# hydradarpa/kalman-hydra

Measured on AMD Instinct MI355X. Metric: frames/sec (Brox flow + EKF update) at 1024^2, higher is better.
Workload: dtype f32 (flow, renders) / f64 (EKF sums and state)

## Files before the change

### kalman-hydra_amd/csrc/chol_flow_kernels.h

```cpp
#pragma once
#include <hip/hip_runtime.h>
#include "dense_kernels.h"

#define FLOW_NT 256
#ifdef HM_STAMP
#define HM_CHAIN_STAMP(c, k) do { if (g_stamp && (threadIdx.x & 63) == 0) g_stamp[(size_t)(4096 + (c)) * 8 + (k)] = clock64(); } while (0)
#else
#define HM_CHAIN_STAMP(c, k) do { } while (0)
#endif
#define FLOW_SENTINEL 0x7FF8DEADBEEF0001ull
#define FLOW_POLL_LIMIT 4000000


__device__ __forceinline__ unsigned long long flow_ld_bits(const double *p)
{
    return __hip_atomic_load((const unsigned long long *)p, __ATOMIC_RELAXED, __HIP_MEMORY_SCOPE_AGENT);
}
__device__ __forceinline__ void flow_st(double *p, double v)
{
    __hip_atomic_store((unsigned long long *)p, (unsigned long long)__double_as_longlong(v), __ATOMIC_RELAXED,
                       __HIP_MEMORY_SCOPE_AGENT);
}

__device__ __forceinline__ void flow_fill_row(const FlowArgs &a, int row, int t, int nt)
{
    const double s = __longlong_as_double((long long)FLOW_SENTINEL);
    if (row < a.nrows) {
        const int upto = row < a.nb * DNB ? (row / DNB) * DNB : a.n;
        for (int j = t; j < upto; j += nt) a.L[(size_t)row * a.n + j] = s;
    }
    if (row < a.n) {
        const int upto = min(a.n, (row / DNB + 1) * DNB);
        for (int j = t; j < upto; j += nt) a.Tinv[(size_t)row * a.n + j] = s;
    }
}
#define FLOW_FILL_WGS 32
__device__ __forceinline__ void flow_fill_blocks(const FlowArgs &a, int t, int nt)
{
    const double s = __longlong_as_double((long long)FLOW_SENTINEL);
    for (int i = t; i < a.nb * DNB * DNB; i += nt) a.Lt[i] = s;
    for (int i = t; i < 3 * a.nb * DNB * DNB; i += nt) a.P[i] = s;
    if (t == 0) a.ctl[0] = 0;
}
__global__ __launch_bounds__(256) void k_flow_fill(FlowArgs a)
{
    if ((int)blockIdx.x >= a.nrows) flow_fill_blocks(a, ((int)blockIdx.x - a.nrows) * 256 + threadIdx.x, 256 * FLOW_FILL_WGS);
    else flow_fill_row(a, blockIdx.x, threadIdx.x, 256);
}

struct FlowBlock {
    const double *src;
    int ld, nr, nc;
    double (*dst)[DNB + 1];
};

__device__ __forceinline__ bool flow_fetch2(const FlowBlock &b0, const FlowBlock &b1, bool two, unsigned *ctl, bool hot = false)
{
    const int t = threadIdx.x;
    __shared__ int s_ok;
    double v0[4], v1[4];
    int patient = 0;
    for (int tries = 0;; tries++) {
        int ok0 = 1, ok1 = 1;
#pragma unroll
        for (int q = 0; q < 4; q++) {
            const int e = t + FLOW_NT * q, i = e / DNB, j = e % DNB;
            unsigned long long x0 = 0, x1 = 0;
            if (i < b0.nr && j < b0.nc) x0 = flow_ld_bits(b0.src + (size_t)i * b0.ld + j);
            if (two && i < b1.nr && j < b1.nc) x1 = flow_ld_bits(b1.src + (size_t)i * b1.ld + j);
            ok0 &= x0 != FLOW_SENTINEL;
// ... 404 lines not shown
```

### kalman-hydra_amd/csrc/ctx.h

```cpp
#pragma once
#include "hm_common.h"
#include "hm_types.h"
#include <chrono>
#include <cmath>
#include <condition_variable>
#include <functional>
#include <mutex>
#include <thread>
#include <vector>

struct Helper {
    std::thread th;
    std::mutex m;
    std::condition_variable cv;
    std::function<int()> job;
    bool posted = false, busy = false, quit = false;
    int rc = HM_OK;
    char err[512] = "";
    void run()
    {
        std::unique_lock<std::mutex> lk(m);
        for (;;) {
            cv.wait(lk, [&] { return quit || posted; });
            if (quit) return;
// ... 209 lines not shown
    long long n4_ticket = 0;
    bool n4_pending = false;
    int newton_fail = 0;
    hipEvent_t ev_n4 = nullptr, ev_pm = nullptr;
    bool n4_ready = false;
    bool chain_pending = false;
    std::vector<double> chain_pred, chain_proj;
    int chain_its = 0, chain_moved = 0;
    double *pin_blk = nullptr;
    std::thread worker;
    bool worker_active;
    int worker_rc;
    char worker_err[512];
    int chol_flow = 1, flow_wgs = 192;
    int flow_stall = 0;
    int speculate = 1;
    double *d_flowP;
    unsigned *d_flowctl;
    hipStream_t stream2;
    hipStream_t stream4 = nullptr;
    hipEvent_t ev_tail = nullptr;
    bool tail_on_stream4 = false;
    int tail_split = 1;
    int *d_nbars, *d_nvoff, *d_nvbar, *d_ninfo;
    double *d_nl0, *d_nX;
    bool newton_ready = false;
    int *d_ids[3];
    int *d_labels;
    int4 *d_lbox;
    double *d_lout;
    std::vector<double> h_lout;
    int2 *d_outline;
    int *d_outline_cnt;
    uint8_t *d_pm_mask;
    uint8_t *d_pm_flag = nullptr;
    uint8_t *d_pm_pruned = nullptr;
    Ccl ccl = {nullptr, nullptr, nullptr, nullptr, nullptr, 0, 0};
    double *d_pm_X = nullptr;
    double *pin_pm = nullptr;
    std::vector<double> pmv;
    int *d_pm_done = nullptr;
    long long pm_ticket = 0;
    bool pm_ready = false;
    bool outline_ready = false;
    const uint8_t *prepared_mask = nullptr;
    hipEvent_t ev_outline = nullptr;
    hipEvent_t ev_m0 = nullptr;
    ViewState view;
    BodyState body;
    StrainState strain;
    RecState rec;
};

static inline hipError_t alloc_targets(HmOwner &own, Targets &t, size_t n)
{
    hipError_t e = own.alloc(&t.acc, n * sizeof(int));
    if (e == hipSuccess) e = own.alloc(&t.fx, n * sizeof(float));
    if (e == hipSuccess) e = own.alloc(&t.fy, n * sizeof(float));
    if (e == hipSuccess) e = own.alloc(&t.cnt, n * sizeof(int));
    return e;
}

static int helper_join(hm_ctx *h)
{
    if (h->helper_used) {
        const int rc = h->helper.wait();
        if (rc != HM_OK) { hm_set_error("%s", h->helper.err); return rc; }
    }
    return HM_OK;
}
// ... 76 lines not shown
    for (int i = 0; i < n_bars; i++) {
        const int p = bars[2 * i], q = bars[2 * i + 1];
        bar[fill[p]] = i; other[fill[p]++] = q;
        bar[fill[q]] = i; other[fill[q]++] = p;
    }
}

static inline void spring_blocks(int n_bars, const int32_t *bars, const double *l0, double kappa, const double *X, double *blk)
{
    for (int i = 0; i < n_bars; i++) {
        const int a = bars[2 * i], b = bars[2 * i + 1];
        const double dx = X[2 * a] - X[2 * b], dy = X[2 * a + 1] - X[2 * b + 1];
        const double l = std::sqrt(dx * dx + dy * dy);
        const double k = kappa * (1.0 - l0[i] / l), c = kappa * l0[i] / (l * l * l);
        blk[3 * i] = k + c * dx * dx; blk[3 * i + 1] = c * dx * dy; blk[3 * i + 2] = k + c * dy * dy;
    }
}

__attribute__((visibility("hidden"))) void ekf_queue_setup_all(hipStream_t st, const Mesh &m, const double *d_X, TriSetup *d_setup);
__attribute__((visibility("hidden"))) void ekf_queue_render(hipStream_t st, const Mesh &m, const double *d_X, const TriSetup *d_setup,
                                                            const Targets &out, const int *d_labels, int *d_ids);
__attribute__((visibility("hidden"))) void ekf_queue_fpft(hipStream_t st, const double *src, double *FP, double *dst, int N,
                                                          const SpringTopo &tp, double a, double s, double eps_F);
__attribute__((visibility("hidden"))) void ekf_queue_chol_flow(hipStream_t st, const FlowArgs &a, int wgs, bool fill);

__attribute__((visibility("hidden"))) int body_map_build(hm_ctx *h);
__attribute__((visibility("hidden"))) int body_stats_queue_add(hm_ctx *h, const uint8_t *d_reg);
__attribute__((visibility("hidden"))) int body_rec_slot(hm_ctx *h, const char *who, uint8_t **dst);
__attribute__((visibility("hidden"))) int body_rec_queue_copy(hm_ctx *h, uint8_t *dst);
```

### kalman-hydra_amd/csrc/ekf.hip

```cpp
#include "ctx.h"
#include "ekf_kernels.h"
#include "dense_kernels.h"
#include "chol_flow_kernels.h"
#include "project_kernels.h"
#include "predict_kernels.h"
#include <algorithm>
#include <atomic>
#include <chrono>
#include <cmath>
#include <cstring>
#include <set>
#include <thread>
#include <utility>
#include <vector>


static int hb_wait(hipStream_t st, const double *blk, size_t first, size_t n, unsigned long long stamp, double *out, const char *who)
{
    const volatile unsigned long long *canary = (const volatile unsigned long long *)blk + 2 * (first + n - 1);
    const auto t_start = std::chrono::steady_clock::now();
    const auto t_yield = t_start + std::chrono::microseconds(700), t_give_up = t_start + std::chrono::milliseconds(20);
    bool polite = false;
    for (int spin = 0;; spin++) {
        if ((canary[0] ^ canary[1]) == stamp && hb_take(blk, first, n, stamp, out)) return HM_OK;
// ... 226 lines not shown
    return HM_OK;
}
#endif

#define TUNE_SET(field) [](hm_ctx *h, long long v) { h->field = (decltype(h->field))v; }
static const struct TuneKey {
    const char *key;
    long long lo, hi;
    int step;
    void (*set)(hm_ctx *, long long);
    const char *must;
} tune_keys[] = {
    {"measure_split", 1, MEAS_VSPLIT_MAX, 1, TUNE_SET(vsplit), nullptr},
    {"edge_split", 1, MEAS_VSPLIT_MAX, 1, TUNE_SET(esplit), nullptr},
    {"chol_flow", 0, 1, 1, TUNE_SET(chol_flow), "must be 0 (one launch per block step) or 1 (one persistent launch)"},
    {"chol_flow_wgs", 2, 2048, 1, TUNE_SET(flow_wgs), "must be in 2..2048 (the chain workgroup and at least one task workgroup)"},
    {"render_rows", 8, 16, 8, TUNE_SET(render_rows), "must be 8 or 16"},
    {"chol_flow_stall", 0, 100000, 1, TUNE_SET(flow_stall), nullptr},
    {"result_delay", 0, 5000, 1, TUNE_SET(result_delay), "must be in 0..5000 (microseconds)"},
    {"tail_async", 0, 1, 1, TUNE_SET(tail_async), "must be 0 or 1"},
    {"tail_split", 0, 1, 1, TUNE_SET(tail_split), "must be 0 or 1"},
    {"newton_fail", 0, 1, 1, TUNE_SET(newton_fail), "must be 0 or 1"},
    {"speculate", 0, 1, 1, TUNE_SET(speculate), "must be 0 or 1"},
    {"body_stats_cap", 1, BODY_STATS_CAP, 1, TUNE_SET(body.stats_cap), nullptr},
    {"body_rec_chunk", 0, INT32_MAX, 1, TUNE_SET(rec.chunk), "must be >= 0 (0: the default size)"},
    {"rec_tp_frames", 1, REC_TP_MAX, 1, TUNE_SET(rec.tp_frames), nullptr},
    {"rec_bl_frames", 1, REC_BL_MAX, 1, TUNE_SET(rec.bl_frames), nullptr},
    {"rec_res_frames", 1, REC_RES_MAX, 1, TUNE_SET(rec.res_frames), nullptr},
    {"rec_map_frames", 1, REC_MAP_MAX, 1, TUNE_SET(rec.map_frames), nullptr},
    {"rec_null_frames", 1, REC_NULL_MAX, 1, TUNE_SET(rec.null_frames), nullptr},
    {"rec_tm_frames", 1, REC_TM_MAX, 1, TUNE_SET(rec.tm_frames), nullptr},
    {"rec_gram_bytes", 64, REC_GRAM_BYTES_MAX, 64, TUNE_SET(rec.gram_bytes), "must be a multiple of 64 in 64..131008"},
    {"rec_scratch_bytes", 1, 1 << 30, 1, TUNE_SET(rec.scr_bytes), nullptr},
    {"rec_ev_bytes", 1, 1ll << 34, 1, TUNE_SET(rec.ev_bytes), nullptr},
};
#undef TUNE_SET
static const TuneKey *tune_find(const char *key)
{
    for (const TuneKey &k : tune_keys)
        if (!strcmp(key, k.key)) return &k;
    return nullptr;
}
static int tune_set(hm_ctx *h, const char *key, long long value)
{
    const TuneKey *k = tune_find(key);
    HM_ARG(k != nullptr, "hm_ctx_tune: unknown key '%s'", key);
// ... 149 lines not shown
    h->prepared_mask = nullptr;
    return HM_OK;
}

static int render_dev(hm_ctx *h, const double *dX, Targets t)
{
    Mesh m = {h->W, h->H, h->N, h->T, h->d_tri, h->d_uv, h->d_tex};
    hipLaunchKernelGGL(k_setup_all, dim3(hm_cdiv(h->T, 64)), dim3(64), 0, h->stream, m, dX, h->d_setup);
    hipLaunchKernelGGL((k_render<0>), dim3(hm_cdiv(h->W, EKF_TILE), hm_cdiv(h->H, EKF_TILE)), dim3(EKF_TILE, EKF_TILE), 0,
                       h->stream, m, dX, h->d_setup, t, (const int *)nullptr, (int *)nullptr);
    HM_HIP(hipGetLastError());
    return HM_OK;
}

static int render_into(hm_ctx *h, const double *X, Targets t)
{
    HM_HIP(hipMemcpyAsync(h->d_X, X, (size_t)4 * h->N * sizeof(double), hipMemcpyHostToDevice, h->stream));
    return render_dev(h, h->d_X, t);
}

static void measure_args(hm_ctx *h, const double *dX, double deltaX, int masked, MeasureArgs &a);
static int render_strips(const hm_ctx *h) { return hm_cdiv(h->W, RI_W) * hm_cdiv(h->H, h->render_rows); }

static int render_iter(hm_ctx *h, const double *dX, Targets t, bool with_err, int masked, bool regions, double deltaX)
{
    IterRenderArgs r;
    r.m = Mesh{h->W, h->H, h->N, h->T, h->d_tri, h->d_uv, h->d_tex};
    r.X = dX;
    r.out = t;
    r.o = Obs{h->o_yim, masked ? h->d_yfxm : h->o_yfx, masked ? h->d_yfym : h->o_yfy, h->o_ym};
    r.raw_fx = h->o_yfx; r.raw_fy = h->o_yfy;
    r.partial = h->d_tpart;
    r.tiles_x = hm_cdiv(h->W, RI_W); r.tiles_y = hm_cdiv(h->H, h->render_rows);
    const int nstrips = r.tiles_x * r.tiles_y;
    r.with_err = with_err ? 1 : 0;
    r.n_regions = regions ? h->N : 0;
    MeasureArgs a;
    measure_args(h, dX, deltaX, masked, a);
    if (h->render_rows == 8) hipLaunchKernelGGL((k_render_iter<8>), dim3(r.n_regions + nstrips), dim3(256), 0, h->stream, r, a, h->d_area);
    else hipLaunchKernelGGL((k_render_iter<16>), dim3(r.n_regions + nstrips), dim3(256), 0, h->stream, r, a, h->d_area);
    HM_HIP(hipGetLastError());
    return HM_OK;
}

static void hm_tile_partial_sums(const double *p, int ntiles, double s[RI_NV])
{
    static thread_local double g[RI_GROUPS][RI_NV];
    for (int t = 0; t < RI_GROUPS; t++) {
        double a[RI_NV];
        for (int k = 0; k < RI_NV; k++) a[k] = 0.0;
        for (int i = t; i < ntiles; i += RI_GROUPS)
            for (int k = 0; k < RI_NV; k++) a[k] += p[RI_NV * (size_t)i + k];
        for (int k = 0; k < RI_NV; k++) g[t][k] = a[k];
    }
    for (int k = 0; k < RI_NV; k++) {
        double v = 0.0;
        for (int t = 0; t < RI_GROUPS; t++) v += g[t][k];
        s[k] = v;
    }
}

#define NEED_TEX(h, who) \
    if (!(h)->have_tex) { hm_set_error(who ": hm_set_texture has not been called"); return HM_ERR_STATE; }
// ... 200 lines not shown
}

extern "C" int hm_error(hm_ctx_t h, const double *X, int masked, double err[4], float *fx, float *fy)
{
    HM_ARG(h && X && err, "hm_error: NULL argument");
    HM_JOIN(h);
    NEED_TEX(h, "hm_error");
    NEED_OBS(h, "hm_error");
    HM_HIP(hipSetDevice(h->device));
    HM_HIP(hipMemcpyAsync(h->d_X, X, (size_t)4 * h->N * sizeof(double), hipMemcpyHostToDevice, h->stream));
    HM_TRY(render_iter(h, h->d_X, h->P, true, masked, false, 2.0));
    const int n = h->W * h->H;
    if (fx) HM_HIP(hipMemcpyAsync(fx, h->P.fx, (size_t)n * sizeof(float), hipMemcpyDeviceToHost, h->stream));
    if (fy) HM_HIP(hipMemcpyAsync(fy, h->P.fy, (size_t)n * sizeof(float), hipMemcpyDeviceToHost, h->stream));
    HM_HIP(hipMemcpyAsync(h->h_tpart.data(), h->d_tpart, (size_t)render_strips(h) * RI_NV * sizeof(double), hipMemcpyDeviceToHost, h->stream));
    HM_HIP(stream_wait(h->stream));
    double s6[RI_NV];
    hm_tile_partial_sums(h->h_tpart.data(), render_strips(h), s6);
    for (int k = 0; k < 4; k++) err[k] = s6[k];
    return HM_OK;
}

static int measure_dev(hm_ctx *h, const double *dX, bool ref_ready, double deltaX, int masked, bool regions_ready = false,
                       bool scatter = true)
{
    if (!ref_ready) {
        HM_TRY(render_iter(h, dX, h->ref, false, masked, !regions_ready, deltaX));
        regions_ready = true;
    }
    MeasureArgs a;
    measure_args(h, dX, deltaX, masked, a);
    if (!regions_ready) hipLaunchKernelGGL(k_star_regions, dim3(h->N), dim3(REGION_NT), 0, h->stream, a, h->d_area);
    hipLaunchKernelGGL(k_measure_vertex, dim3(h->N, h->vsplit), dim3(MEAS_NT), 0, h->stream, a,
                       (const TriSetup *)h->d_cfgs, (const int4 *)h->d_ubox, (const unsigned *)h->d_tmask);
    if (h->E > 0) hipLaunchKernelGGL(k_measure_edge, dim3(h->E, h->esplit), dim3(MEAS_NT), 0, h->stream, a);
    if (scatter) {
        ScatterArgs s = {h->d_out, h->d_edges, h->N, h->E, h->vsplit, h->esplit, h->eps_Z, h->eps_J, h->eps_M, deltaX, h->d_HTH, h->d_Hz, h->d_Hzc};
        hipLaunchKernelGGL(k_hth_scatter, dim3(hm_cdiv(h->njobs, 4)), dim3(256), 0, h->stream, s);
    }
    HM_HIP(hipGetLastError());
    return HM_OK;
}

static void measure_args(hm_ctx *h, const double *dX, double deltaX, int masked, MeasureArgs &a)
{
    a.m = Mesh{h->W, h->H, h->N, h->T, h->d_tri, h->d_uv, h->d_tex};
    a.topo = StarTopo{h->d_star_off, h->d_star_tri, h->d_edges, h->E};
    a.ref = h->ref;
    a.obs = obs_of(h, masked);
    a.X = dX;
    a.delta = deltaX;
    a.out = h->d_out;
    a.pool = h->pool;
    a.vsplit = h->vsplit;
    a.esplit = h->esplit;
    a.iZ = 1.0 / h->eps_Z; a.iJ = 1.0 / h->eps_J; a.iM = 1.0 / h->eps_M;
    a.cfgs = h->d_cfgs;
    a.ubox = h->d_ubox;
    a.tmask = h->d_tmask;
    a.tlist = h->d_tlist;
    a.tcount = h->d_tcount;
// ... 17 lines not shown
    NEED_OBS(h, "hm_measure");
    HM_HIP(hipSetDevice(h->device));
    const size_t n4 = (size_t)4 * h->N;
    int *ovf = h->pin_scratch;
    for (int attempt = 0;; attempt++) {
        HM_TRY(measure_on_device(h, X, deltaX, masked));
        *ovf = 0;
        HM_HIP(hipMemcpyAsync(ovf, h->pool.overflow, sizeof(int), hipMemcpyDeviceToHost, h->stream));
        HM_HIP(hipStreamSynchronize(h->stream));
        if (!*ovf) break;
        if (attempt) { hm_set_error("hm_measure: the star regions do not fit the difference-image pool"); return HM_ERR_STATE; }
        HM_TRY(pool_grow(h, "hm_measure"));
    }
    HM_HIP(hipMemcpyAsync(Hz, h->d_Hz, n4 * sizeof(double), hipMemcpyDeviceToHost, h->stream));
    if (Hzc) HM_HIP(hipMemcpyAsync(Hzc, h->d_Hzc, n4 * 4 * sizeof(double), hipMemcpyDeviceToHost, h->stream));
    HM_HIP(hipMemcpyAsync(HTH, h->d_HTH, n4 * n4 * sizeof(double), hipMemcpyDeviceToHost, h->stream));
    HM_HIP(hipStreamSynchronize(h->stream));
    return HM_OK;
}

static int aug_rows(int n) { return hm_cdiv(n, DNB) * DNB + DNB; }

static void chol_factor(hm_ctx *h, double *A, double *L, double *Lt, double *T, double *M, int n, bool with_rhs,
                        bool first_done = false, hipStream_t st = nullptr)
{
    if (!st) st = h->stream;
    const int nb = hm_cdiv(n, DNB);
    const int nrows = with_rhs ? aug_rows(n) : n;
    const int nbr = hm_cdiv(nrows, DNB);
    if (h->chol_flow) {
        ekf_queue_chol_flow(st, FlowArgs{A, L, Lt, T, h->d_flowP, n, nrows, nb, nbr, h->d_flowctl, h->flow_stall}, h->flow_wgs, !first_done);
        return;
    }
    if (!first_done) hipLaunchKernelGGL(k_chol_first, dim3(1), dim3(64), 0, st, A, Lt, n);
    for (int k = 0; k < nb; k++) {
        const int mr = nbr - k - 1, mc = std::max(nb - k - 1, 1);
        hipLaunchKernelGGL(k_chol_step, dim3((mc + k + 1) * (mr + 1)), dim3(256), 0, st, A, L, Lt, T, M, n, nrows, nb, k, mc, mc + k + 1, mr + 1);
    }
}

static void chol_inverse(hm_ctx *h, int n, const double *T, double *out, hipStream_t st = nullptr)
{
    const int nb = hm_cdiv(n, DNB);
    hipLaunchKernelGGL(k_ttt, dim3(nb, nb), dim3(256), 0, st ? st : h->stream, T, n, out);
}

static int flow_status(hm_ctx *h, const char *who)
{
    if (!h->chol_flow) return HM_OK;
    unsigned ctl[2] = {0, 0};
    HM_HIP(hipMemcpyAsync(ctl, h->d_flowctl, sizeof ctl, hipMemcpyDeviceToHost, h->stream));
    HM_HIP(hipStreamSynchronize(h->stream));
    if (ctl[1]) { hm_set_error("%s: the factorisation launch gave up waiting for a block (chol_flow time-out)", who); return HM_ERR_HIP; }
    return HM_OK;
// ... 15 lines not shown
        p.A = A; p.Hz = h->d_Hz; p.Hzc = h->d_Hzc; p.n = n4; p.rhs_row = rhs_index;
        p.f = FlowArgs{A, h->d_Af[slot], h->d_Lt[slot], h->d_T[slot], h->d_flowP, n4, nrows, nb, hm_cdiv(nrows, DNB), h->d_flowctl, 0};
        hipLaunchKernelGGL(k_solve_prep, dim3(nrows + FLOW_FILL_WGS), dim3(256), 0, h->stream, p);
    }
    if (h->d_Wres == h->d_Wtmp) h->d_Wres = nullptr;
    chol_factor(h, A, h->d_Af[slot], h->d_Lt[slot], h->d_T[slot], h->d_Wtmp, n4, true, h->chol_flow != 0);
    const double *yrow = h->d_Af[slot] + (rhs_row - A);
    hipLaunchKernelGGL(k_tvec, dim3(hm_cdiv(n4, TV_COLS)), dim3(TV_COLS * TV_ROWS), 0, h->stream, h->d_T[slot], n4, yrow, h->d_step, h->d_X0,
                       h->d_Xn);
    return h->d_step;
}

static int prior_inverse(hm_ctx *h, const double *W_prior, hipStream_t st = nullptr)
{
    if (!st) st = h->stream;
    const int n4 = 4 * h->N;
    const size_t nnb = (size_t)n4 * n4 * sizeof(double);
    if (W_prior)
        HM_HIP(hipMemcpyAsync(h->d_Wprior, W_prior, nnb, hipMemcpyHostToDevice, st));
    else if (h->d_Wres != h->d_Wprior)
        HM_HIP(hipMemcpyAsync(h->d_Wprior, h->d_Wres, nnb, hipMemcpyDeviceToDevice, st));
    if (!h->chol_flow) HM_HIP(hipMemcpyAsync(h->d_Awork, h->d_Wprior, nnb, hipMemcpyDeviceToDevice, st));
    h->d_Wres = h->d_Wprior;
    HM_HIP(hipMemsetAsync(h->d_flowctl, 0, 4 * sizeof(unsigned), st));
    chol_factor(h, h->chol_flow ? h->d_Wprior : h->d_Awork, h->d_Af[0], h->d_Lt[0], h->d_Wtmp, h->d_invW0, n4, false, false, st);
    chol_inverse(h, n4, h->d_Wtmp, h->d_invW0, st);
    HM_HIP(hipGetLastError());
    return HM_OK;
}

extern "C" int hm_update_prefactor(hm_ctx_t h)
{
    HM_ARG(h != nullptr, "hm_update_prefactor: NULL handle");
    HM_JOIN(h);
    if (!h->d_Wres) { hm_set_error("hm_update_prefactor: no covariance resident on the device"); return HM_ERR_STATE; }
    HM_HIP(hipSetDevice(h->device));
    h->pq_valid = false;
    if (h->chol_flow) {
        const int rc = prior_inverse(h, nullptr);
        if (rc == HM_OK) {
            h->prefactored = true;
            h->upd_open = false;
        }
        return rc;
    }
    h->worker_active = true;
    h->worker = std::thread([h]() {
        int rc = hipSetDevice(h->device) == hipSuccess ? HM_OK : HM_ERR_HIP;
// ... 195 lines not shown

extern "C" int hm_update_arm_newton(hm_ctx_t h, void *worker, int n_bars, const int32_t *bars, const double *l0, double kappa,
                                    double M, double dt, int maxiter, double tol)
{
    HM_ARG(h && worker && n_bars >= 0 && bars && l0, "hm_update_arm_newton: bad argument");
    HM_JOIN_LAZY(h);
    h->armed.worker = worker;
    h->pn_bars.assign(bars, bars + 2 * (size_t)n_bars);
    h->pn_l0.assign(l0, l0 + n_bars);
    h->pn_par[0] = kappa; h->pn_par[1] = M; h->pn_par[2] = dt; h->pn_par[3] = tol;
    h->pn_maxiter = maxiter;
    h->armed.newton = true;
    return HM_OK;
}

extern "C" int hm_update_arm_cov(hm_ctx_t h, double eps_F)
{
    HM_ARG(h != nullptr, "hm_update_arm_cov: NULL handle");
    h->armed.cov = true;
    h->pq_eps_F = eps_F;
    return HM_OK;
}

static int queue_predict_ahead(hm_ctx *h, const double *X, int n_bars, const int32_t *bars, const double *l0, double kappa,
                               double M, double dt, double eps_F, hipStream_t st);
static int prepare_mask(hm_ctx *h, const uint8_t *d_y_m);

extern "C" int hm_update_arm_mask(hm_ctx_t h, const uint8_t *d_y_m)
{
    HM_ARG(h != nullptr, "hm_update_arm_mask: NULL handle");
    h->armed.mask = d_y_m;
    return HM_OK;
}

extern "C" int hm_update_tail(hm_ctx_t h, double *Hzc, double *gains)
{
    HM_ARG(h != nullptr, "hm_update_tail: NULL handle");
    HM_JOIN_LAZY(h);
    if (!h->tail_valid) {
        hm_set_error("hm_update_tail: the last hm_update_run on this handle did not succeed (or there was none)");
        return HM_ERR_STATE;
    }
    const size_t n4 = (size_t)4 * h->N;
    if (h->tail_pending) {
        HM_HIP(hipSetDevice(h->device));
        HM_TRY(hb_wait(h->tail_stream, h->pin + 2 * (n4 + RES_HEAD), 0, n4 * 7, hb_stamp(h->tail_ticket), h->tailv.data(), "hm_update_tail"));
// ... 6 lines not shown

struct UpdateArgs {
    const double *W_prior;
    double *X;
    double deltaX;
    int masked, max_iter;
    double reltol;
    double *errs, *Hzc, *gains, *W_out;
};
struct UpdateRun {
    hm_ctx *const h;
    const UpdateArgs a;
    const Armed armed;
    const uint8_t *next_mask;
    const int n4;
    bool chained = false, collected = false;
    std::vector<double> X0, Xcur, Xold;
    int niter = 0, accepted = 0;
    bool reverted = false, conv = false;
    bool ref_ready = false;
    bool regions_ahead = false;
    bool measured_ahead = false;
    bool grown = false;
    double eold = 0.0;
    int slot = 0;
    bool dbg = false;
    std::chrono::steady_clock::time_point t_enter, t_queued;
    double stage[5] = {0, 0, 0, 0, 0};

    UpdateRun(hm_ctx *h, const UpdateArgs &a)
        : h(h), a(a), armed(std::exchange(h->armed, {})), next_mask(armed.mask), n4(4 * h->N) {}
    double ms() const { return std::chrono::duration<double, std::milli>(std::chrono::steady_clock::now() - t_enter).count(); }
    const double *res() const { return h->resv.data(); }
    double *pin_tail() const { return h->pin + 2 * ((size_t)n4 + RES_HEAD); }
};

struct SpecSwap {
    hm_ctx *const h;
    bool swapped = false;
    explicit SpecSwap(hm_ctx *h) : h(h) {}
    SpecSwap(const SpecSwap &) = delete;
    SpecSwap &operator=(const SpecSwap &) = delete;
    ~SpecSwap() { undo(); }
    void flip() { std::swap(h->ref, h->P); std::swap(h->d_X, h->d_Xn); }
    void set() { flip(); swapped = true; }
    void undo() { if (swapped) flip(); swapped = false; }
// ... 15 lines not shown
    if (h->n4v[n4 + 1] != 0.0) return 2;
    u.X0 = h->chain_proj; u.Xcur = u.X0; u.Xold = u.X0;
    h->upd_X0 = u.X0;
    h->X0 = u.X0;
    u.collected = true;
    return HM_OK;
}

static int update_enter(UpdateRun &u)
{
    hm_ctx *h = u.h;
    h->tail_valid = false;
    HM_JOIN_LAZY(h);
    HM_ARG(u.a.deltaX > 0 && u.a.max_iter >= 0, "hm_update_run: deltaX must be positive, max_iter >= 0");
    u.chained = h->chain_pending;
    h->chain_pending = false;
    h->last_err_valid = false;
    h->pq_valid = false;
    h->tail_pending = false;
    NEED_TEX(h, "hm_update_run");
    NEED_OBS(h, "hm_update_run");
    u.dbg = getenv("HYDRA_MI_TRACE") != nullptr;
    u.t_enter = std::chrono::steady_clock::now();
    HM_TRY(update_begin(h, u.a.W_prior, u.chained ? nullptr : u.a.X));
    u.stage[0] = u.ms();
    u.collected = !u.chained;
    if (!u.chained) {
        u.X0.assign(u.a.X, u.a.X + u.n4); u.Xcur = u.X0; u.Xold = u.X0;
        HM_HIP(hipMemcpyAsync(h->d_X, h->d_X0, (size_t)u.n4 * sizeof(double), hipMemcpyDeviceToDevice, h->stream));
    }
    return HM_OK;
}

static int update_queue_iteration(UpdateRun &u, int it, SpecSwap &swap)
{
    hm_ctx *h = u.h;
    if (!u.measured_ahead) HM_TRY(measure_dev(h, h->d_X, u.ref_ready, u.a.deltaX, u.a.masked, u.regions_ahead, false));
    u.measured_ahead = false;
    if (u.next_mask && it == 0) {
        HM_HIP(h->own.event(&h->ev_m0));
        HM_HIP(hipEventRecord(h->ev_m0, h->stream));
    }
    if (u.collected) h->X0 = u.Xcur;
    h->have_ref = true;
    u.slot = h->upd_last == 0 ? 1 : 0;
    HM_TRY(ctx_join(h));
    double *rhs_row = solve_step(h, u.slot, u.a.deltaX);
    u.regions_ahead = it + 1 < u.a.max_iter;
    HM_TRY(render_iter(h, h->d_Xn, h->P, true, u.a.masked, u.regions_ahead, u.a.deltaX));
    hipLaunchKernelGGL(k_iter_result, dim3(1), dim3(256), 0, h->stream, rhs_row, u.n4, h->d_tpart,
                       render_strips(h), h->pool.overflow, (const unsigned *)h->d_flowctl, h->pin, (double)(++h->run_ticket),
                       h->result_delay);
    HM_HIP(hipGetLastError());
    if (h->speculate && u.regions_ahead) {
        swap.set();
        u.measured_ahead = true;
        HM_TRY(measure_dev(h, h->d_X, true, u.a.deltaX, u.a.masked, true, false));
    }
    u.t_queued = std::chrono::steady_clock::now();
    return HM_OK;
}

static int update_meanwhile(UpdateRun &u, int it)
{
    hm_ctx *h = u.h;
    if (u.next_mask && it == 0) {
        HM_TRY(ensure_stream2(h));
        HM_HIP(hipStreamWaitEvent(h->stream2, h->ev_m0, 0));
        HM_TRY(prepare_mask(h, u.next_mask));
// ... 87 lines not shown
    u.ref_ready = true;
    h->X0 = u.Xcur;
    *out = Verdict::go_on;
    return HM_OK;
}

static int update_state_final(UpdateRun &u)
{
    hm_ctx *h = u.h;
    if (!u.collected) HM_TRY(chain_collect(u));
    u.stage[1] = u.ms();
    if (u.armed.newton)
        HM_TRY(hm_ms_newton_start(u.armed.worker, h->N, (int)h->pn_l0.size(), h->pn_bars.data(), h->pn_l0.data(), h->pn_par[0],
                                  h->pn_par[1], h->pn_par[2], h->pn_maxiter, h->pn_par[3], u.Xcur.data()));
    u.stage[2] = u.ms();
    return HM_OK;
}

struct TailJob {
    hm_ctx *h;
    const uint8_t *next_mask;
    int which;
    hipStream_t ts;
    int niter, n4;
    double *pin_tail;
    long long ticket;
    double *W_out;
    bool ahead;
    double eps_F;
};
static int tail_launches(const TailJob &j, const std::vector<double> &Xk)
{
    hm_ctx *h = j.h;
    const int n4 = j.n4;
    HM_HIP(hipSetDevice(h->device));
    if (j.next_mask) HM_TRY(prepare_mask(h, j.next_mask));
    HM_TRY(update_cov_on(h, j.which, nullptr, j.ts));
    if (j.niter > 0) {
        hipLaunchKernelGGL(k_gains, dim3(n4), dim3(256), 0, j.ts, h->d_Wres, h->d_Hzc, n4, h->d_gain);
        hipLaunchKernelGGL(k_tail_result, dim3(1), dim3(1024), 0, j.ts, h->d_Hzc, h->d_gain, n4, j.pin_tail, (double)j.ticket,
                           h->result_delay);
    }
    if (j.W_out) HM_HIP(hipMemcpyAsync(j.W_out, h->d_Wres, (size_t)n4 * n4 * sizeof(double), hipMemcpyDeviceToHost, j.ts));
    HM_HIP(hipGetLastError());
    if (j.ahead)
        HM_TRY(queue_predict_ahead(h, Xk.data(), (int)h->pn_l0.size(), h->pn_bars.data(), h->pn_l0.data(), h->pn_par[0],
                                   h->pn_par[1], h->pn_par[2], j.eps_F, j.ts));
    if (j.ts != h->stream) {
        HM_HIP(hipEventRecord(h->ev_tail, j.ts));
        h->tail_on_stream4 = true;
    }
    return HM_OK;
}

static int update_tail(UpdateRun &u)
{
    hm_ctx *h = u.h;
    const int n4 = u.n4;
    int which = -1;
    if (u.reverted) which = u.accepted == 0 ? -1 : 1;
    else which = u.niter == 0 ? -1 : 0;
    hipStream_t ts = h->stream;
    HM_TRY(ctx_join(h));
    if (!u.a.W_out && h->tail_split) {
        HM_HIP(h->own.stream(&h->stream4));
        HM_HIP(h->own.event(&h->ev_tail));
        ts = h->stream4;
    }
    const long long ticket = u.niter > 0 ? ++h->run_ticket : h->run_ticket;
    const bool ahead = u.armed.cov && u.armed.newton && h->chol_flow && which >= 0 && u.niter > 0 && !u.a.W_out;
    const TailJob job = {h, u.next_mask, which, ts, u.niter, n4, u.pin_tail(), ticket, u.a.W_out, ahead, h->pq_eps_F};
    u.stage[3] = u.ms();
    if (u.niter > 0 && !u.a.W_out && !u.a.Hzc && !u.a.gains) {
        h->tail_pending = true;
        h->tail_ticket = ticket;
        h->tail_stream = ts;
        if (h->tail_async) {
            h->helper_used = true;
            h->helper.post([job, Xk = u.Xcur]() { return tail_launches(job, Xk); });
        } else {
            HM_TRY(tail_launches(job, u.Xcur));
        }
    } else if (u.niter > 0 && !u.a.W_out) {
        HM_TRY(tail_launches(job, u.Xcur));
        HM_TRY(hb_wait(ts, job.pin_tail, 0, (size_t)n4 * 7, hb_stamp(ticket), h->tailv.data(), "hm_update_run"));
    } else {
        HM_TRY(tail_launches(job, u.Xcur));
        HM_HIP(stream_wait(ts));
        if (u.niter > 0 && !hb_take(job.pin_tail, 0, (size_t)n4 * 7, hb_stamp(ticket), h->tailv.data())) {
            hm_set_error("hm_update_run: the gains did not arrive although the stream has completed");
            return HM_ERR_HIP;
        }
    }
    u.stage[4] = u.ms();
    if (u.dbg && u.stage[4] > 5.0)
        fprintf(stderr, "[hydra_mi] hm_update_run %d iterations: begin %.2f loop-end %.2f newton-started %.2f tail-queued %.2f tail-done %.2f ms\n",
                u.niter, u.stage[0], u.stage[1], u.stage[2], u.stage[3], u.stage[4]);
    return HM_OK;
}

static void update_finish(UpdateRun &u, int info[4])
{
    hm_ctx *h = u.h;
    const size_t n4 = u.n4;
    if (u.niter > 0) {
        if (u.a.Hzc) memcpy(u.a.Hzc, h->tailv.data(), n4 * 4 * sizeof(double));
        if (u.a.gains) memcpy(u.a.gains, h->tailv.data() + n4 * 4, n4 * 3 * sizeof(double));
    } else {
        if (u.a.Hzc) memset(u.a.Hzc, 0, n4 * 4 * sizeof(double));
        if (u.a.gains) memset(u.a.gains, 0, n4 * 3 * sizeof(double));
        std::fill(h->tailv.begin(), h->tailv.end(), 0.0);
    }
    h->tail_valid = true;
    memcpy(u.a.X, u.Xcur.data(), n4 * sizeof(double));
    info[0] = u.niter; info[1] = u.accepted; info[2] = u.reverted ? 1 : 0; info[3] = u.conv ? 1 : 0;
    if (u.niter > 0 && !u.reverted) {
        const double *res = u.res();
        h->last_err[0] = res[n4]; h->last_err[1] = res[n4 + 8]; h->last_err[2] = res[n4 + 9]; h->last_err[3] = res[n4 + 3];
        h->last_err_X = u.Xcur;
        h->last_err_valid = true;
    }
}

extern "C" int hm_update_run(hm_ctx_t h, const double *W_prior, double *X, double deltaX, int masked, int max_iter,
                             double reltol, int info[4], double *errs, double *Hzc, double *gains, double *W_out)
{
    HM_ARG(h && X && info, "hm_update_run: NULL argument");
    UpdateRun u(h, {W_prior, X, deltaX, masked, max_iter, reltol, errs, Hzc, gains, W_out});
    HM_TRY(update_enter(u));
    for (int it = 0; it < max_iter;) {
        SpecSwap swap(h);
        HM_TRY(update_queue_iteration(u, it, swap));
        HM_TRY(update_meanwhile(u, it));
        Taken taken = Taken::go_on;
        HM_TRY(update_take_result(u, it, swap, &taken));
        if (taken == Taken::retry) continue;
        Verdict verdict = Verdict::go_on;
        HM_TRY(update_judge(u, it, &verdict));
        if (verdict != Verdict::go_on) break;
        swap.keep();
        it++;
    }
    HM_TRY(update_state_final(u));
    HM_TRY(update_tail(u));
    update_finish(u, info);
    return HM_OK;
}

extern "C" int hm_update_last_error(hm_ctx_t h, const double *X, double err[4])
{
    HM_ARG(h && X && err, "hm_update_last_error: NULL argument");
    if (!h->last_err_valid || h->last_err_X.size() != (size_t)4 * h->N) return 1;
    if (memcmp(X, h->last_err_X.data(), (size_t)4 * h->N * sizeof(double)) != 0) return 1;
    for (int k = 0; k < 4; k++) err[k] = h->last_err[k];
    return HM_OK;
}

void ekf_queue_fpft(hipStream_t st, const double *src, double *FP, double *dst, int N, const SpringTopo &tp, double a, double s,
                    double eps_F)
{
    const dim3 grid(hm_cdiv(4 * N, 256), N);
    hipLaunchKernelGGL(k_fw_rows, grid, dim3(256), 0, st, src, FP, N, tp, a, s);
    hipLaunchKernelGGL(k_pft_cols, grid, dim3(256), 0, st, (const double *)FP, dst, N, tp, a, s, eps_F);
}
void ekf_queue_chol_flow(hipStream_t st, const FlowArgs &a, int wgs, bool fill)
{
    if (fill) hipLaunchKernelGGL(k_flow_fill, dim3(a.nrows + FLOW_FILL_WGS), dim3(256), 0, st, a);
    hipLaunchKernelGGL(k_chol_flow, dim3(wgs), dim3(FLOW_NT), 0, st, a);
}

static int cov_predict_core(hm_ctx *h, const double *W_in, int n_bars, const int32_t *bars, const double *blocks,
                            double a, double s, double eps_F, double *W_out, bool ahead, hipStream_t st = nullptr)
{
    if (!st) st = h->stream;
    const int N = h->N, n4 = 4 * N;
    const size_t nn = (size_t)n4 * n4 * sizeof(double);
    std::vector<int> &off = h->sp_h_off, &bar = h->sp_h_bar, &other = h->sp_h_other;
    if (!ahead) HM_HIP(stream_wait(st));
    const bool same_topo = h->d_sp_off && h->sp_bars_cached.size() == 2 * (size_t)n_bars &&
                           (n_bars == 0 || memcmp(h->sp_bars_cached.data(), bars, 2 * (size_t)n_bars * sizeof(int32_t)) == 0);
    if (!same_topo) {
        for (int i = 0; i < n_bars; i++)
            HM_ARG(bars[2 * i] >= 0 && bars[2 * i] < N && bars[2 * i + 1] >= 0 && bars[2 * i + 1] < N,
                   "hm_cov_predict: spring %d refers to a vertex outside 0..%d", i, N - 1);
        spring_csr(N, n_bars, bars, off, bar, other);
        HM_HIP(h->own.alloc(&h->d_sp_off, (size_t)(N + 1) * sizeof(int)));
        HM_HIP(h->own.grow(&h->d_sp_bar, 2 * (size_t)n_bars * sizeof(int)));
        HM_HIP(h->own.grow(&h->d_sp_other, 2 * (size_t)n_bars * sizeof(int)));
        HM_HIP(h->own.grow(&h->d_sp_blk, 3 * (size_t)n_bars * sizeof(double)));
        HM_HIP(hipMemcpyAsync(h->d_sp_off, off.data(), (size_t)(N + 1) * sizeof(int), hipMemcpyHostToDevice, st));
        if (n_bars > 0) {
            HM_HIP(hipMemcpyAsync(h->d_sp_bar, bar.data(), bar.size() * sizeof(int), hipMemcpyHostToDevice, st));
            HM_HIP(hipMemcpyAsync(h->d_sp_other, other.data(), other.size() * sizeof(int), hipMemcpyHostToDevice, st));
        }
        h->sp_bars_cached.assign(bars, bars + 2 * (size_t)n_bars);
    }
    if (n_bars > 0) {
        const double *from = blocks;
        if (!ahead) {
            h->sp_h_blk.assign(blocks, blocks + 3 * (size_t)n_bars);
            from = h->sp_h_blk.data();
        }
        HM_HIP(hipMemcpyAsync(h->d_sp_blk, from, 3 * (size_t)n_bars * sizeof(double), hipMemcpyHostToDevice, st));
    }
    const double *src = h->d_Wres;
    if (W_in) {
        HM_HIP(hipMemcpyAsync(h->d_H, W_in, nn, hipMemcpyHostToDevice, st));
        src = h->d_H;
    } else if (src == h->d_Wtmp) {
        HM_HIP(hipMemcpyAsync(h->d_H, h->d_Wtmp, nn, hipMemcpyDeviceToDevice, st));
        src = h->d_H;
    }
    SpringTopo tp = {h->d_sp_off, h->d_sp_bar, h->d_sp_other, h->d_sp_blk};
    ekf_queue_fpft(st, src, h->d_Awork, ahead ? h->d_Wprior : h->d_Wtmp, N, tp, a, s, eps_F);
    HM_HIP(hipGetLastError());
    if (ahead) return HM_OK;
    if (W_out) HM_HIP(hipMemcpyAsync(W_out, h->d_Wtmp, nn, hipMemcpyDeviceToHost, st));
    if (W_out) HM_HIP(stream_wait(st));
    h->d_Wres = h->d_Wtmp;
    h->prefactored = false;
    return HM_OK;
}

extern "C" int hm_cov_predict(hm_ctx_t h, const double *W_in, int n_bars, const int32_t *bars, const double *blocks,
                              double a, double s, double eps_F, double *W_out)
{
    HM_ARG(h && n_bars >= 0 && (n_bars == 0 || (bars && blocks)), "hm_cov_predict: bad argument");
    HM_JOIN(h);
    if (!W_in && !h->d_Wres) {
        hm_set_error("hm_cov_predict: no covariance given and none resident on the device");
        return HM_ERR_STATE;
    }
    HM_HIP(hipSetDevice(h->device));
    h->pq_valid = false;
    return cov_predict_core(h, W_in, n_bars, bars, blocks, a, s, eps_F, W_out, false);
}

static int queue_predict_ahead(hm_ctx *h, const double *X, int n_bars, const int32_t *bars, const double *l0, double kappa,
                               double M, double dt, double eps_F, hipStream_t st)
{
    for (int i = 0; i < 2 * n_bars; i++)
        if (bars[i] < 0 || bars[i] >= h->N) return HM_OK;
    HM_HIP(h->own.host_grow(&h->pin_blk, 3 * (size_t)n_bars * sizeof(double), hipHostMallocDefault));
    spring_blocks(n_bars, bars, l0, kappa, X, h->pin_blk);
    double *const post = h->d_Wres;
    HM_TRY(cov_predict_core(h, nullptr, n_bars, bars, h->pin_blk, dt, dt / M, eps_F, nullptr, true, st));
    h->d_Wres = h->d_Wprior;
    const int rc = prior_inverse(h, nullptr, st);
    h->d_Wres = post;
    if (rc) return rc;
    h->upd_open = false;
    h->pq_X.assign(X, X + 4 * (size_t)h->N);
    h->pq_bars.assign(bars, bars + 2 * (size_t)n_bars);
    h->pq_l0.assign(l0, l0 + n_bars);
    h->pq_par[0] = kappa; h->pq_par[1] = dt; h->pq_par[2] = dt / M; h->pq_par[3] = eps_F;
    h->pq_valid = true;
    return HM_OK;
}

extern "C" int hm_predict_take(hm_ctx_t h, const double *X, int n_bars, const int32_t *bars, const double *l0, double kappa,
                               double a, double s, double eps_F)
{
    HM_ARG(h && X && n_bars >= 0 && (n_bars == 0 || (bars && l0)), "hm_predict_take: bad argument");
    HM_JOIN_LAZY(h);
    if (!h->pq_valid) return 1;
    h->pq_valid = false;
    const size_t n4 = (size_t)4 * h->N;
// ... 230 lines not shown
```

Measured before the change: 333.9.

## Overlap first measurement and gains with covariance chain on side streams

Runs the first iteration's measurement on a secondary stream gated by an event, so it can proceed alongside the chained covariance work, and joins back before the solve. In the tail, gains and the result kernel move to the main stream after a covariance event, while the predict-ahead runs on the tail stream concurrently. Spring blocks are now uploaded before the covariance update. The flow-control memset is folded into the fill kernel via a 'fresh' flag. This adds cross-stream event dependencies and possible ordering hazards on shared buffers.

After: 336.8 (median of 6 runs). Within noise of the previous version (+0.9%).

```diff
diff --git a/kalman-hydra_amd/csrc/chol_flow_kernels.h b/kalman-hydra_amd/csrc/chol_flow_kernels.h
--- a/kalman-hydra_amd/csrc/chol_flow_kernels.h
+++ b/kalman-hydra_amd/csrc/chol_flow_kernels.h
@@ -42,10 +42,14 @@
     for (int i = t; i < 3 * a.nb * DNB * DNB; i += nt) a.P[i] = s;
     if (t == 0) a.ctl[0] = 0;
 }
-__global__ __launch_bounds__(256) void k_flow_fill(FlowArgs a)
-{
-    if ((int)blockIdx.x >= a.nrows) flow_fill_blocks(a, ((int)blockIdx.x - a.nrows) * 256 + threadIdx.x, 256 * FLOW_FILL_WGS);
-    else flow_fill_row(a, blockIdx.x, threadIdx.x, 256);
+__global__ __launch_bounds__(256) void k_flow_fill(FlowArgs a, int fresh)
+{
+    if ((int)blockIdx.x >= a.nrows) {
+        flow_fill_blocks(a, ((int)blockIdx.x - a.nrows) * 256 + threadIdx.x, 256 * FLOW_FILL_WGS);
+        if (fresh && (int)blockIdx.x == a.nrows && threadIdx.x == 0) a.ctl[1] = 0;
+    } else {
+        flow_fill_row(a, blockIdx.x, threadIdx.x, 256);
+    }
 }
 
 struct FlowBlock {
diff --git a/kalman-hydra_amd/csrc/ctx.h b/kalman-hydra_amd/csrc/ctx.h
--- a/kalman-hydra_amd/csrc/ctx.h
+++ b/kalman-hydra_amd/csrc/ctx.h
@@ -255,6 +255,7 @@
     hipEvent_t ev_tail = nullptr;
     bool tail_on_stream4 = false;
     int tail_split = 1;
+    hipEvent_t ev_cov = nullptr;
     int *d_nbars, *d_nvoff, *d_nvbar, *d_ninfo;
     double *d_nl0, *d_nX;
     bool newton_ready = false;
@@ -279,6 +280,8 @@
     const uint8_t *prepared_mask = nullptr;
     hipEvent_t ev_outline = nullptr;
     hipEvent_t ev_m0 = nullptr;
+    int first_on_chain = 1;
+    hipEvent_t ev_first_in = nullptr, ev_first_out = nullptr;
     ViewState view;
     BodyState body;
     StrainState strain;
@@ -401,7 +404,7 @@
                                                             const Targets &out, const int *d_labels, int *d_ids);
 __attribute__((visibility("hidden"))) void ekf_queue_fpft(hipStream_t st, const double *src, double *FP, double *dst, int N,
                                                           const SpringTopo &tp, double a, double s, double eps_F);
-__attribute__((visibility("hidden"))) void ekf_queue_chol_flow(hipStream_t st, const FlowArgs &a, int wgs, bool fill);
+__attribute__((visibility("hidden"))) void ekf_queue_chol_flow(hipStream_t st, const FlowArgs &a, int wgs, bool fill, bool fresh = false);
 
 __attribute__((visibility("hidden"))) int body_map_build(hm_ctx *h);
 __attribute__((visibility("hidden"))) int body_stats_queue_add(hm_ctx *h, const uint8_t *d_reg);
diff --git a/kalman-hydra_amd/csrc/ekf.hip b/kalman-hydra_amd/csrc/ekf.hip
--- a/kalman-hydra_amd/csrc/ekf.hip
+++ b/kalman-hydra_amd/csrc/ekf.hip
@@ -272,6 +272,7 @@
     {"tail_split", 0, 1, 1, TUNE_SET(tail_split), "must be 0 or 1"},
     {"newton_fail", 0, 1, 1, TUNE_SET(newton_fail), "must be 0 or 1"},
     {"speculate", 0, 1, 1, TUNE_SET(speculate), "must be 0 or 1"},
+    {"first_on_chain", 0, 1, 1, TUNE_SET(first_on_chain), "must be 0 or 1"},
     {"body_stats_cap", 1, BODY_STATS_CAP, 1, TUNE_SET(body.stats_cap), nullptr},
     {"body_rec_chunk", 0, INT32_MAX, 1, TUNE_SET(rec.chunk), "must be >= 0 (0: the default size)"},
     {"rec_tp_frames", 1, REC_TP_MAX, 1, TUNE_SET(rec.tp_frames), nullptr},
@@ -467,8 +468,10 @@
 static void measure_args(hm_ctx *h, const double *dX, double deltaX, int masked, MeasureArgs &a);
 static int render_strips(const hm_ctx *h) { return hm_cdiv(h->W, RI_W) * hm_cdiv(h->H, h->render_rows); }
 
-static int render_iter(hm_ctx *h, const double *dX, Targets t, bool with_err, int masked, bool regions, double deltaX)
-{
+static int render_iter(hm_ctx *h, const double *dX, Targets t, bool with_err, int masked, bool regions, double deltaX,
+                       hipStream_t st = nullptr)
+{
+    if (!st) st = h->stream;
     IterRenderArgs r;
     r.m = Mesh{h->W, h->H, h->N, h->T, h->d_tri, h->d_uv, h->d_tex};
     r.X = dX;
@@ -482,8 +485,8 @@
     r.n_regions = regions ? h->N : 0;
     MeasureArgs a;
     measure_args(h, dX, deltaX, masked, a);
-    if (h->render_rows == 8) hipLaunchKernelGGL((k_render_iter<8>), dim3(r.n_regions + nstrips), dim3(256), 0, h->stream, r, a, h->d_area);
-    else hipLaunchKernelGGL((k_render_iter<16>), dim3(r.n_regions + nstrips), dim3(256), 0, h->stream, r, a, h->d_area);
+    if (h->render_rows == 8) hipLaunchKernelGGL((k_render_iter<8>), dim3(r.n_regions + nstrips), dim3(256), 0, st, r, a, h->d_area);
+    else hipLaunchKernelGGL((k_render_iter<16>), dim3(r.n_regions + nstrips), dim3(256), 0, st, r, a, h->d_area);
     HM_HIP(hipGetLastError());
     return HM_OK;
 }
@@ -730,21 +733,22 @@
 }
 
 static int measure_dev(hm_ctx *h, const double *dX, bool ref_ready, double deltaX, int masked, bool regions_ready = false,
-                       bool scatter = true)
-{
+                       bool scatter = true, hipStream_t st = nullptr)
+{
+    if (!st) st = h->stream;
     if (!ref_ready) {
-        HM_TRY(render_iter(h, dX, h->ref, false, masked, !regions_ready, deltaX));
+        HM_TRY(render_iter(h, dX, h->ref, false, masked, !regions_ready, deltaX, st));
         regions_ready = true;
     }
     MeasureArgs a;
     measure_args(h, dX, deltaX, masked, a);
-    if (!regions_ready) hipLaunchKernelGGL(k_star_regions, dim3(h->N), dim3(REGION_NT), 0, h->stream, a, h->d_area);
-    hipLaunchKernelGGL(k_measure_vertex, dim3(h->N, h->vsplit), dim3(MEAS_NT), 0, h->stream, a,
+    if (!regions_ready) hipLaunchKernelGGL(k_star_regions, dim3(h->N), dim3(REGION_NT), 0, st, a, h->d_area);
+    hipLaunchKernelGGL(k_measure_vertex, dim3(h->N, h->vsplit), dim3(MEAS_NT), 0, st, a,
                        (const TriSetup *)h->d_cfgs, (const int4 *)h->d_ubox, (const unsigned *)h->d_tmask);
-    if (h->E > 0) hipLaunchKernelGGL(k_measure_edge, dim3(h->E, h->esplit), dim3(MEAS_NT), 0, h->stream, a);
+    if (h->E > 0) hipLaunchKernelGGL(k_measure_edge, dim3(h->E, h->esplit), dim3(MEAS_NT), 0, st, a);
     if (scatter) {
         ScatterArgs s = {h->d_out, h->d_edges, h->N, h->E, h->vsplit, h->esplit, h->eps_Z, h->eps_J, h->eps_M, deltaX, h->d_HTH, h->d_Hz, h->d_Hzc};
-        hipLaunchKernelGGL(k_hth_scatter, dim3(hm_cdiv(h->njobs, 4)), dim3(256), 0, h->stream, s);
+        hipLaunchKernelGGL(k_hth_scatter, dim3(hm_cdiv(h->njobs, 4)), dim3(256), 0, st, s);
     }
     HM_HIP(hipGetLastError());
     return HM_OK;
@@ -808,14 +812,15 @@
 static int aug_rows(int n) { return hm_cdiv(n, DNB) * DNB + DNB; }
 
 static void chol_factor(hm_ctx *h, double *A, double *L, double *Lt, double *T, double *M, int n, bool with_rhs,
-                        bool first_done = false, hipStream_t st = nullptr)
+                        bool first_done = false, hipStream_t st = nullptr, bool fresh = false)
 {
     if (!st) st = h->stream;
     const int nb = hm_cdiv(n, DNB);
     const int nrows = with_rhs ? aug_rows(n) : n;
     const int nbr = hm_cdiv(nrows, DNB);
     if (h->chol_flow) {
-        ekf_queue_chol_flow(st, FlowArgs{A, L, Lt, T, h->d_flowP, n, nrows, nb, nbr, h->d_flowctl, h->flow_stall}, h->flow_wgs, !first_done);
+        ekf_queue_chol_flow(st, FlowArgs{A, L, Lt, T, h->d_flowP, n, nrows, nb, nbr, h->d_flowctl, h->flow_stall}, h->flow_wgs, !first_done,
+                            fresh && !first_done);
         return;
     }
     if (!first_done) hipLaunchKernelGGL(k_chol_first, dim3(1), dim3(64), 0, st, A, Lt, n);
@@ -877,8 +882,8 @@
         HM_HIP(hipMemcpyAsync(h->d_Wprior, h->d_Wres, nnb, hipMemcpyDeviceToDevice, st));
     if (!h->chol_flow) HM_HIP(hipMemcpyAsync(h->d_Awork, h->d_Wprior, nnb, hipMemcpyDeviceToDevice, st));
     h->d_Wres = h->d_Wprior;
-    HM_HIP(hipMemsetAsync(h->d_flowctl, 0, 4 * sizeof(unsigned), st));
-    chol_factor(h, h->chol_flow ? h->d_Wprior : h->d_Awork, h->d_Af[0], h->d_Lt[0], h->d_Wtmp, h->d_invW0, n4, false, false, st);
+    if (!h->chol_flow) HM_HIP(hipMemsetAsync(h->d_flowctl, 0, 4 * sizeof(unsigned), st));
+    chol_factor(h, h->chol_flow ? h->d_Wprior : h->d_Awork, h->d_Af[0], h->d_Lt[0], h->d_Wtmp, h->d_invW0, n4, false, false, st, true);
     chol_inverse(h, n4, h->d_Wtmp, h->d_invW0, st);
     HM_HIP(hipGetLastError());
     return HM_OK;
@@ -1120,6 +1125,8 @@
     return HM_OK;
 }
 
+static int predict_ahead_springs(hm_ctx *h, const double *X, int n_bars, const int32_t *bars, const double *l0, double kappa,
+                                 hipStream_t st, bool *go);
 static int queue_predict_ahead(hm_ctx *h, const double *X, int n_bars, const int32_t *bars, const double *l0, double kappa,
                                double M, double dt, double eps_F, hipStream_t st);
 static int prepare_mask(hm_ctx *h, const uint8_t *d_y_m);
@@ -1172,6 +1179,8 @@
     bool regions_ahead = false;
     bool measured_ahead = false;
     bool grown = false;
+    bool first_on_chain = false;
+    bool first_in_flight = false;
     double eold = 0.0;
     int slot = 0;
     bool dbg = false;
@@ -1233,6 +1242,13 @@
     NEED_OBS(h, "hm_update_run");
     u.dbg = getenv("HYDRA_MI_TRACE") != nullptr;
     u.t_enter = std::chrono::steady_clock::now();
+    if (u.chained && h->first_on_chain && u.a.max_iter > 0) {
+        HM_HIP(hipSetDevice(h->device));
+        HM_HIP(h->own.event(&h->ev_first_in));
+        HM_HIP(h->own.event(&h->ev_first_out));
+        HM_HIP(hipEventRecord(h->ev_first_in, h->stream));
+        u.first_on_chain = true;
+    }
     HM_TRY(update_begin(h, u.a.W_prior, u.chained ? nullptr : u.a.X));
     u.stage[0] = u.ms();
     u.collected = !u.chained;
@@ -1246,16 +1262,28 @@
 static int update_queue_iteration(UpdateRun &u, int it, SpecSwap &swap)
 {
     hm_ctx *h = u.h;
-    if (!u.measured_ahead) HM_TRY(measure_dev(h, h->d_X, u.ref_ready, u.a.deltaX, u.a.masked, u.regions_ahead, false));
+    hipStream_t ms = h->stream;
+    if (u.first_on_chain && it == 0 && !u.measured_ahead) {
+        ms = h->stream3;
+        HM_HIP(hipStreamWaitEvent(ms, h->ev_first_in, 0));
+        u.first_in_flight = true;
+    }
+    u.first_on_chain = false;
+    if (!u.measured_ahead) HM_TRY(measure_dev(h, h->d_X, u.ref_ready, u.a.deltaX, u.a.masked, u.regions_ahead, false, ms));
     u.measured_ahead = false;
+    if (ms != h->stream) HM_HIP(hipEventRecord(h->ev_first_out, ms));
     if (u.next_mask && it == 0) {
         HM_HIP(h->own.event(&h->ev_m0));
-        HM_HIP(hipEventRecord(h->ev_m0, h->stream));
+        HM_HIP(hipEventRecord(h->ev_m0, ms));
     }
     if (u.collected) h->X0 = u.Xcur;
     h->have_ref = true;
     u.slot = h->upd_last == 0 ? 1 : 0;
     HM_TRY(ctx_join(h));
+    if (ms != h->stream) {
+        HM_HIP(hipStreamWaitEvent(h->stream, h->ev_first_out, 0));
+        u.first_in_flight = false;
+    }
     double *rhs_row = solve_step(h, u.slot, u.a.deltaX);
     u.regions_ahead = it + 1 < u.a.max_iter;
     HM_TRY(render_iter(h, h->d_Xn, h->P, true, u.a.masked, u.regions_ahead, u.a.deltaX));
@@ -1389,6 +1417,7 @@
     const uint8_t *next_mask;
     int which;
     hipStream_t ts;
+    hipStream_t gs;
     int niter, n4;
     double *pin_tail;
     long long ticket;
@@ -1401,22 +1430,39 @@
     hm_ctx *h = j.h;
     const int n4 = j.n4;
     HM_HIP(hipSetDevice(h->device));
+    bool ahead = false;
+    if (j.ahead)
+        HM_TRY(predict_ahead_springs(h, Xk.data(), (int)h->pn_l0.size(), h->pn_bars.data(), h->pn_l0.data(), h->pn_par[0], j.ts, &ahead));
+    HM_TRY(update_cov_on(h, j.which, nullptr, j.ts));
     if (j.next_mask) HM_TRY(prepare_mask(h, j.next_mask));
-    HM_TRY(update_cov_on(h, j.which, nullptr, j.ts));
-    if (j.niter > 0) {
-        hipLaunchKernelGGL(k_gains, dim3(n4), dim3(256), 0, j.ts, h->d_Wres, h->d_Hzc, n4, h->d_gain);
-        hipLaunchKernelGGL(k_tail_result, dim3(1), dim3(1024), 0, j.ts, h->d_Hzc, h->d_gain, n4, j.pin_tail, (double)j.ticket,
-                           h->result_delay);
-    }
-    if (j.W_out) HM_HIP(hipMemcpyAsync(j.W_out, h->d_Wres, (size_t)n4 * n4 * sizeof(double), hipMemcpyDeviceToHost, j.ts));
-    HM_HIP(hipGetLastError());
-    if (j.ahead)
-        HM_TRY(queue_predict_ahead(h, Xk.data(), (int)h->pn_l0.size(), h->pn_bars.data(), h->pn_l0.data(), h->pn_par[0],
-                                   h->pn_par[1], h->pn_par[2], j.eps_F, j.ts));
-    if (j.ts != h->stream) {
+    const bool beside = j.gs != j.ts;
+    auto predict = [&]() -> int {
+        if (!ahead) return HM_OK;
+        return queue_predict_ahead(h, Xk.data(), (int)h->pn_l0.size(), h->pn_bars.data(), h->pn_l0.data(), h->pn_par[0],
+                                   h->pn_par[1], h->pn_par[2], j.eps_F, j.ts);
+    };
+    auto gains = [&]() -> int {
+        if (j.niter > 0) {
+            hipLaunchKernelGGL(k_gains, dim3(n4), dim3(256), 0, j.gs, h->d_Wres, h->d_Hzc, n4, h->d_gain);
+            hipLaunchKernelGGL(k_tail_result, dim3(1), dim3(1024), 0, j.gs, h->d_Hzc, h->d_gain, n4, j.pin_tail, (double)j.ticket,
+                               h->result_delay);
+        }
+        if (j.W_out) HM_HIP(hipMemcpyAsync(j.W_out, h->d_Wres, (size_t)n4 * n4 * sizeof(double), hipMemcpyDeviceToHost, j.ts));
+        HM_HIP(hipGetLastError());
+        return HM_OK;
+    };
+    if (beside) {
+        HM_HIP(hipEventRecord(h->ev_cov, j.ts));
+        HM_TRY(predict());
         HM_HIP(hipEventRecord(h->ev_tail, j.ts));
-        h->tail_on_stream4 = true;
-    }
+        HM_HIP(hipStreamWaitEvent(j.gs, h->ev_cov, 0));
+        HM_TRY(gains());
+    } else {
+        HM_TRY(gains());
+        HM_TRY(predict());
+        if (j.ts != h->stream) HM_HIP(hipEventRecord(h->ev_tail, j.ts));
+    }
+    if (j.ts != h->stream) h->tail_on_stream4 = true;
     return HM_OK;
 }
 
@@ -1436,12 +1482,17 @@
     }
     const long long ticket = u.niter > 0 ? ++h->run_ticket : h->run_ticket;
     const bool ahead = u.armed.cov && u.armed.newton && h->chol_flow && which >= 0 && u.niter > 0 && !u.a.W_out;
-    const TailJob job = {h, u.next_mask, which, ts, u.niter, n4, u.pin_tail(), ticket, u.a.W_out, ahead, h->pq_eps_F};
+    hipStream_t gs = ts;
+    if (ahead && ts != h->stream) {
+        HM_HIP(h->own.event(&h->ev_cov));
+        gs = h->stream;
+    }
+    const TailJob job = {h, u.next_mask, which, ts, gs, u.niter, n4, u.pin_tail(), ticket, u.a.W_out, ahead, h->pq_eps_F};
     u.stage[3] = u.ms();
     if (u.niter > 0 && !u.a.W_out && !u.a.Hzc && !u.a.gains) {
         h->tail_pending = true;
         h->tail_ticket = ticket;
-        h->tail_stream = ts;
+        h->tail_stream = gs;
         if (h->tail_async) {
             h->helper_used = true;
             h->helper.post([job, Xk = u.Xcur]() { return tail_launches(job, Xk); });
@@ -1450,7 +1501,7 @@
         }
     } else if (u.niter > 0 && !u.a.W_out) {
         HM_TRY(tail_launches(job, u.Xcur));
-        HM_TRY(hb_wait(ts, job.pin_tail, 0, (size_t)n4 * 7, hb_stamp(ticket), h->tailv.data(), "hm_update_run"));
+        HM_TRY(hb_wait(gs, job.pin_tail, 0, (size_t)n4 * 7, hb_stamp(ticket), h->tailv.data(), "hm_update_run"));
     } else {
         HM_TRY(tail_launches(job, u.Xcur));
         HM_HIP(stream_wait(ts));
@@ -1497,7 +1548,10 @@
     HM_TRY(update_enter(u));
     for (int it = 0; it < max_iter;) {
         SpecSwap swap(h);
-        HM_TRY(update_queue_iteration(u, it, swap));
+        if (const int rc = update_queue_iteration(u, it, swap)) {
+            if (u.first_in_flight) (void)hipStreamSynchronize(h->stream3);
+            return rc;
+        }
         HM_TRY(update_meanwhile(u, it));
         Taken taken = Taken::go_on;
         HM_TRY(update_take_result(u, it, swap, &taken));
@@ -1530,18 +1584,15 @@
     hipLaunchKernelGGL(k_fw_rows, grid, dim3(256), 0, st, src, FP, N, tp, a, s);
     hipLaunchKernelGGL(k_pft_cols, grid, dim3(256), 0, st, (const double *)FP, dst, N, tp, a, s, eps_F);
 }
-void ekf_queue_chol_flow(hipStream_t st, const FlowArgs &a, int wgs, bool fill)
-{
-    if (fill) hipLaunchKernelGGL(k_flow_fill, dim3(a.nrows + FLOW_FILL_WGS), dim3(256), 0, st, a);
+void ekf_queue_chol_flow(hipStream_t st, const FlowArgs &a, int wgs, bool fill, bool fresh)
+{
+    if (fill) hipLaunchKernelGGL(k_flow_fill, dim3(a.nrows + FLOW_FILL_WGS), dim3(256), 0, st, a, fresh ? 1 : 0);
     hipLaunchKernelGGL(k_chol_flow, dim3(wgs), dim3(FLOW_NT), 0, st, a);
 }
 
-static int cov_predict_core(hm_ctx *h, const double *W_in, int n_bars, const int32_t *bars, const double *blocks,
-                            double a, double s, double eps_F, double *W_out, bool ahead, hipStream_t st = nullptr)
-{
-    if (!st) st = h->stream;
-    const int N = h->N, n4 = 4 * N;
-    const size_t nn = (size_t)n4 * n4 * sizeof(double);
+static int spring_upload(hm_ctx *h, int n_bars, const int32_t *bars, const double *blocks, bool ahead, hipStream_t st)
+{
+    const int N = h->N;
     std::vector<int> &off = h->sp_h_off, &bar = h->sp_h_bar, &other = h->sp_h_other;
     if (!ahead) HM_HIP(stream_wait(st));
     const bool same_topo = h->d_sp_off && h->sp_bars_cached.size() == 2 * (size_t)n_bars &&
@@ -1570,6 +1621,16 @@
         }
         HM_HIP(hipMemcpyAsync(h->d_sp_blk, from, 3 * (size_t)n_bars * sizeof(double), hipMemcpyHostToDevice, st));
     }
+    return HM_OK;
+}
+
+static int cov_predict_core(hm_ctx *h, const double *W_in, int n_bars, const int32_t *bars, const double *blocks,
+                            double a, double s, double eps_F, double *W_out, bool ahead, hipStream_t st = nullptr)
+{
+    if (!st) st = h->stream;
+    const int N = h->N, n4 = 4 * N;
+    const size_t nn = (size_t)n4 * n4 * sizeof(double);
+    if (!ahead) HM_TRY(spring_upload(h, n_bars, bars, blocks, false, st));
     const double *src = h->d_Wres;
     if (W_in) {
         HM_HIP(hipMemcpyAsync(h->d_H, W_in, nn, hipMemcpyHostToDevice, st));
@@ -1603,13 +1664,21 @@
     return cov_predict_core(h, W_in, n_bars, bars, blocks, a, s, eps_F, W_out, false);
 }
 
-static int queue_predict_ahead(hm_ctx *h, const double *X, int n_bars, const int32_t *bars, const double *l0, double kappa,
-                               double M, double dt, double eps_F, hipStream_t st)
-{
+static int predict_ahead_springs(hm_ctx *h, const double *X, int n_bars, const int32_t *bars, const double *l0, double kappa,
+                                 hipStream_t st, bool *go)
+{
+    *go = false;
     for (int i = 0; i < 2 * n_bars; i++)
         if (bars[i] < 0 || bars[i] >= h->N) return HM_OK;
     HM_HIP(h->own.host_grow(&h->pin_blk, 3 * (size_t)n_bars * sizeof(double), hipHostMallocDefault));
     spring_blocks(n_bars, bars, l0, kappa, X, h->pin_blk);
+    HM_TRY(spring_upload(h, n_bars, bars, h->pin_blk, true, st));
+    *go = true;
+    return HM_OK;
+}
+static int queue_predict_ahead(hm_ctx *h, const double *X, int n_bars, const int32_t *bars, const double *l0, double kappa,
+                               double M, double dt, double eps_F, hipStream_t st)
+{
     double *const post = h->d_Wres;
     HM_TRY(cov_predict_core(h, nullptr, n_bars, bars, h->pin_blk, dt, dt / M, eps_F, nullptr, true, st));
     h->d_Wres = h->d_Wprior;
```
